# microsoft/protnote

Hardware: AMD Instinct MI355X
Metric: protein-label pairs/sec (fwd+bwd) (higher is better)
Workload: dtype f32

## Files before the change

### include/protnote_hip.h

```cpp
#ifndef PROTNOTE_HIP_H
#define PROTNOTE_HIP_H

#include <stddef.h>
#include <stdint.h>

#ifdef __cplusplus
extern "C" {
#endif

#define PN_MAX_BLOCKS 16
#define PN_MAX_LAYERS 8
#define PN_LABEL_F32 0
#define PN_LABEL_I64 1
#define PN_LABEL_U8 2

const char* pn_last_error(void);
int pn_version(void);
const char* pn_build_hash(void);

typedef struct pn_bn {
  const float* weight;
  const float* bias;
  float* running_mean;
  float* running_var;
// ... 179 lines not shown

#define PN_ADAM_WS_BYTES 32768
int pn_clip_adam_step(float* w, const float* g, float* m, float* v, long n, float max_norm, float lr, float beta1,
                      float beta2, float eps, float weight_decay, int step, float* norm_out, void* ws,
                      size_t ws_bytes, void* stream);

int pn_clip_sgd_step(float* w, const float* g, float* momentum_buf, long n, float max_norm, float lr, float momentum,
                     float weight_decay, int step, float* norm_out, void* ws, size_t ws_bytes, void* stream);

int pn_transpose(const float* src, long ld_src, int rows, int cols, float* dst, long ld_dst, void* stream);

int pn_gemm_tn(const float* A, long lda, const float* Bm, long ldb, float* C, long ldc, long R, int M, int N,
               void* ws, size_t ws_bytes, void* stream);

int pn_onehot_batch(const uint8_t* ids, const int64_t* offsets, int B, int A, int Lmax, float* onehots,
                    int64_t* lengths, void* stream);


int pn_ap_append(const float* scores, int ld_s, const void* labels, int label_kind, int ld_y, int B, int N_L,
                 uint32_t* keys, uint8_t* hits, long long cap, long long n0, void* stream);
size_t pn_ap_ws_bytes(int N_L, long long n, long long cap, int micro);
int pn_ap_compute(const uint32_t* keys, const uint8_t* hits, int N_L, long long n, long long cap, double* ap,
                  long long* npos, double* micro_ap, long long* micro_npos, void* ws, size_t ws_bytes, void* stream);

size_t pn_ap_partial_ws_bytes(long long m);
int pn_ap_partial(const uint32_t* keys, const uint8_t* hits, long long m, long long tp_before, long long k_before,
                  double* partial, long long* npos, void* ws, size_t ws_bytes, void* stream);

int pn_binned_hist_update(const float* scores, int ld_s, const void* labels, int label_kind, int ld_y, int B, int N_L,
                          const float* thresholds, int T, unsigned long long* pos_hist, unsigned long long* all_hist,
                          void* stream);
int pn_binned_auprc(unsigned long long* pos_hist, unsigned long long* all_hist, int N_L, int T, double* out,
                    long long* npos, int with_micro, void* stream);

int pn_set_math_mode(int mode);

int pn_set_mlp_materialize(int on);

typedef int (*pn_sync_hook)(long n_doubles, void* user);
int pn_set_sync_bn(pn_sync_hook hook, void* user, double* stage, long stage_doubles, int world);
int pn_get_math_mode(void);

int pn_set_backward_math(int mode);
int pn_get_backward_math(void);

int pn_set_forward_math(int mode);
int pn_get_forward_math(void);
int pn_set_fwd_staged(int on);
int pn_set_bf16_mfma16(int on);
int pn_set_bwd_deep(int mask);

int pn_set_f32_dma(int on);
int pn_set_b3_dma(int on);

int pn_set_encoder_f64(int on);

int pn_set_conv1_gather(int on);

int pn_dropout_mask(unsigned seed, int stream, float p, long rows, int cols, float* out, void* stream_);

int pn_prof_begin(void);
int pn_prof_end(int max_kinds, int* kinds, long* counts, double* total_ms, double* total_flops);

size_t pn_gemm_nt_stats_ws_bytes(int M, int N);
int pn_gemm_nt(const float* A, long lda, const float* W, long ldw, float* C, long ldc, int M, int N, int K,
               const float* bias, const float* a_scale, const float* a_shift, double* col_sum,
               double* col_sumsq, int tile_variant, void* ws, size_t ws_bytes, void* stream);

#ifdef __cplusplus
}
#endif
#endif
```

### protnote_amd/_lib.py

```python
import ctypes as C
import os

import torch

_HERE = os.path.dirname(os.path.abspath(__file__))
LIB_PATH = os.path.join(_HERE, "libprotnote_hip.so")

PN_MAX_BLOCKS = 16
PN_MAX_LAYERS = 8
PN_ADAM_WS_BYTES = 32768
fp = C.POINTER(C.c_float)


class pn_bn(C.Structure):
    _fields_ = [("weight", C.c_void_p), ("bias", C.c_void_p), ("running_mean", C.c_void_p),
                ("running_var", C.c_void_p)]


class pn_res_block(C.Structure):
    _fields_ = [("bn1", pn_bn), ("conv_a_w", C.c_void_p), ("conv_a_b", C.c_void_p), ("bn2", pn_bn),
                ("conv_b_w", C.c_void_p), ("conv_b_b", C.c_void_p)]


class pn_encoder(C.Structure):
# ... 108 lines not shown
    "pn_loss_fwd_bwd": (C.c_int, [C.c_void_p, C.c_void_p, C.c_void_p, C.c_int, C.c_int, C.c_int, C.c_float,
                                  C.c_float, C.c_float, C.c_float, C.c_float, C.c_void_p, C.c_void_p, C.c_void_p,
                                  C.c_void_p, C.c_void_p, C.c_int, C.c_void_p, C.c_float, C.c_void_p, C.c_size_t,
                                  C.c_void_p]),
    "pn_loss_fwd_bwd_t": (C.c_int, [C.c_void_p, C.c_void_p, C.c_int, C.c_int, C.c_int, C.c_int, C.c_float,
                                    C.c_float, C.c_float, C.c_float, C.c_float, C.c_void_p, C.c_void_p, C.c_void_p,
                                    C.c_void_p, C.c_void_p, C.c_int, C.c_void_p, C.c_float, C.c_void_p, C.c_size_t,
                                    C.c_void_p]),
    "pn_tp_fn_fp_t": (C.c_int, [C.c_void_p, C.c_void_p, C.c_int, C.c_int, C.c_int, C.c_float, C.c_void_p,
                                C.c_void_p, C.c_void_p, C.c_void_p]),
    "pn_supcon_ws_bytes": (C.c_size_t, [C.c_int]),
    "pn_supcon_fwd_bwd": (C.c_int, [C.c_void_p, C.c_void_p, C.c_void_p, C.c_int, C.c_int, C.c_void_p, C.c_void_p,
                                    C.c_void_p, C.c_size_t, C.c_void_p]),
    "pn_tp_fn_fp": (C.c_int, [C.c_void_p, C.c_void_p, C.c_void_p, C.c_int, C.c_int, C.c_float, C.c_void_p,
                              C.c_void_p, C.c_void_p, C.c_void_p]),
    "pn_clip_adam_step": (C.c_int, [C.c_void_p, C.c_void_p, C.c_void_p, C.c_void_p, C.c_long, C.c_float, C.c_float,
                                    C.c_float, C.c_float, C.c_float, C.c_float, C.c_int, C.c_void_p, C.c_void_p,
                                    C.c_size_t, C.c_void_p]),
    "pn_clip_sgd_step": (C.c_int, [C.c_void_p, C.c_void_p, C.c_void_p, C.c_long, C.c_float, C.c_float, C.c_float,
                                   C.c_float, C.c_int, C.c_void_p, C.c_void_p, C.c_size_t, C.c_void_p]),
    "pn_transpose": (C.c_int, [C.c_void_p, C.c_long, C.c_int, C.c_int, C.c_void_p, C.c_long, C.c_void_p]),
    "pn_gemm_tn": (C.c_int, [C.c_void_p, C.c_long, C.c_void_p, C.c_long, C.c_void_p, C.c_long, C.c_long, C.c_int,
                             C.c_int, C.c_void_p, C.c_size_t, C.c_void_p]),
    "pn_onehot_batch": (C.c_int, [C.c_void_p, C.c_void_p, C.c_int, C.c_int, C.c_int, C.c_void_p, C.c_void_p,
                                  C.c_void_p]),
    "pn_ap_append": (C.c_int, [C.c_void_p, C.c_int, C.c_void_p, C.c_int, C.c_int, C.c_int, C.c_int, C.c_void_p,
                               C.c_void_p, C.c_longlong, C.c_longlong, C.c_void_p]),
    "pn_ap_ws_bytes": (C.c_size_t, [C.c_int, C.c_longlong, C.c_longlong, C.c_int]),
    "pn_ap_compute": (C.c_int, [C.c_void_p, C.c_void_p, C.c_int, C.c_longlong, C.c_longlong, C.c_void_p, C.c_void_p,
                                C.c_void_p, C.c_void_p, C.c_void_p, C.c_size_t, C.c_void_p]),
    "pn_ap_partial_ws_bytes": (C.c_size_t, [C.c_longlong]),
    "pn_ap_partial": (C.c_int, [C.c_void_p, C.c_void_p, C.c_longlong, C.c_longlong, C.c_longlong, C.c_void_p, C.c_void_p,
                                C.c_void_p, C.c_size_t, C.c_void_p]),
    "pn_binned_hist_update": (C.c_int, [C.c_void_p, C.c_int, C.c_void_p, C.c_int, C.c_int, C.c_int, C.c_int,
                                        C.c_void_p, C.c_int, C.c_void_p, C.c_void_p, C.c_void_p]),
    "pn_binned_auprc": (C.c_int, [C.c_void_p, C.c_void_p, C.c_int, C.c_int, C.c_void_p, C.c_void_p, C.c_int,
                                  C.c_void_p]),
    "pn_dropout_mask": (C.c_int, [C.c_uint, C.c_int, C.c_float, C.c_long, C.c_int, C.c_void_p, C.c_void_p]),
    "pn_set_math_mode": (C.c_int, [C.c_int]),
    "pn_set_mlp_materialize": (C.c_int, [C.c_int]),
    "pn_set_sync_bn": (C.c_int, [C.c_void_p, C.c_void_p, C.c_void_p, C.c_long, C.c_int]),
    "pn_get_math_mode": (C.c_int, []),
    "pn_set_backward_math": (C.c_int, [C.c_int]),
    "pn_get_backward_math": (C.c_int, []),
    "pn_set_forward_math": (C.c_int, [C.c_int]),
    "pn_get_forward_math": (C.c_int, []),
    "pn_set_fwd_staged": (C.c_int, [C.c_int]),
    "pn_set_bf16_mfma16": (C.c_int, [C.c_int]),
    "pn_set_bwd_deep": (C.c_int, [C.c_int]),
    "pn_set_f32_dma": (C.c_int, [C.c_int]),
    "pn_set_encoder_f64": (C.c_int, [C.c_int]),
    "pn_set_conv1_gather": (C.c_int, [C.c_int]),
    "pn_set_b3_dma": (C.c_int, [C.c_int]),
    "pn_prof_begin": (C.c_int, []),
    "pn_prof_end": (C.c_int, [C.c_int, C.POINTER(C.c_int), C.POINTER(C.c_long), C.POINTER(C.c_double),
                              C.POINTER(C.c_double)]),
    "pn_gemm_nt": (C.c_int, [C.c_void_p, C.c_long, C.c_void_p, C.c_long, C.c_void_p, C.c_long, C.c_int, C.c_int,
                             C.c_int, C.c_void_p, C.c_void_p, C.c_void_p, C.c_void_p, C.c_void_p, C.c_int,
                             C.c_void_p, C.c_size_t, C.c_void_p]),
    "pn_gemm_nt_stats_ws_bytes": (C.c_size_t, [C.c_int, C.c_int]),
    "pn_loss_ws_bytes": (C.c_size_t, [C.c_int, C.c_int]),
}


def exported_symbols():
    return sorted(_SIGS)


def _ensure_current():
    from . import build

    have_src = os.path.isdir(build.CSRC) and os.path.exists(os.path.join(build.CSRC, "protnote_hip.hip"))
    if os.path.exists(LIB_PATH) and (not have_src or os.environ.get("PN_SKIP_HASH_CHECK") == "1"):
        return
    if os.path.exists(LIB_PATH) and not build.stale():
        return
    why = "is missing" if not os.path.exists(LIB_PATH) else (
        f"was built from other sources (binary {build.embedded_hash()}, csrc/ {build.csrc_hash()})")
    if not build.have_hipcc():
        raise RuntimeError(f"{LIB_PATH} {why} and hipcc is not available to rebuild it; build it with "
                           "`python -m protnote_amd.build` (protnote_amd has no CPU/eager fallback)")
    try:
        build.build_lib(verbose=False)
    except Exception as exc:
        raise RuntimeError(f"{LIB_PATH} {why} and could not be rebuilt ({exc}); build it with "
                           "`python -m protnote_amd.build` (protnote_amd has no CPU/eager fallback)") from exc


def build_hash() -> str:
    return lib().pn_build_hash().decode()


def lib():
    global _lib
    if _lib is None:
        _ensure_current()
        l = C.CDLL(LIB_PATH)
        for name, (res, args) in _SIGS.items():
            fn = getattr(l, name)
            fn.restype = res
            fn.argtypes = args
        _lib = l
        mode = os.environ.get("PN_MATH_MODE")
        if mode:
            set_math_mode(mode)
        mode = os.environ.get("PN_BACKWARD_MATH")
# ... 135 lines not shown
```

### protnote_amd/csrc/abi_heads_eval.hpp

```cpp
extern "C" size_t pn_mlp_rows_ws_bytes(const pn_mlp* m, int rows) {
  size_t b = 0;
  int hmax = 0;
  for (int i = 0; i + 1 < m->nlayers; ++i) hmax = m->dims[i + 1] > hmax ? m->dims[i + 1] : hmax;
  b += 2 * al256((size_t)rows * hmax * sizeof(float));
  b += 2 * al256((size_t)hmax * sizeof(float));
  return b;
}

extern "C" int pn_mlp_rows_fwd_eval(const pn_mlp* m, const float* x, int ldx, int rows, float* y, void* ws,
                                    size_t ws_bytes, void* stream) {
  PN_OK(math_field_check(m->math_mode, "pn_mlp_rows_fwd_eval"));
  MathScope math_scope(m->math_mode);
  hipStream_t st = (hipStream_t)stream;
  if (m->nlayers < 1 || m->nlayers > PN_MAX_LAYERS) return fail("mlp: bad layer count %d", m->nlayers);
  for (int i = 0; i <= m->nlayers; ++i)
    if (i < m->nlayers && m->dims[i] % 4 != 0) return fail("mlp: dims[%d]=%d not a multiple of 4", i, m->dims[i]);
  if (ldx % 4 != 0) return fail("mlp: ldx %% 4 != 0");
  int hmax = 0;
  for (int i = 0; i + 1 < m->nlayers; ++i) hmax = m->dims[i + 1] > hmax ? m->dims[i + 1] : hmax;
  Bump bp(ws, ws_bytes);
  float* buf[2];
  buf[0] = bp.take<float>((size_t)rows * hmax);
  buf[1] = bp.take<float>((size_t)rows * hmax);
  float* s = bp.take<float>(hmax);
// ... 442 lines not shown
    long rps = (p.R + ns - 1) / ns;
    p.rows_per_split = (rps + 31) / 32 * 32;
    ns = (int)((p.R + p.rows_per_split - 1) / p.rows_per_split);
  }
  const unsigned tiles = (unsigned)((p.M / 256) * (p.N / 256));
  dim3 grid(tiles, (unsigned)ns);
  p.task_ns = 0;
  int* sync_ws = p.task_sync;
  p.task_sync = nullptr;
  if (p.M == 3072 && p.N == 3072 && ns >= 2) {
    p.task_ns = ns;
    grid = dim3(tn_task_grid(ns), 1);
    if (SYNC && sync_ws != nullptr && ns * 4 * 4 <= TN_SYNC_INTS) {
      HIP_OK(hipMemsetAsync(sync_ws, 0, (size_t)ns * 4 * 4 * sizeof(int), st));
      p.task_sync = sync_ws;
    }
  }
  {
    ProfScope ps(100 + TA_PLAIN * 10 + TB, 2.0 * (double)R_all * (double)p.M * (double)p.N, st);
    hipLaunchKernelGGL(kern, grid, dim3(512), TN_FAST_LDS_BYTES, st, p);
    if (tail != 0) {
      auto tk = gemm_tn_kernel<TA_PLAIN, TB, false>;
      static bool tattr[64] = {false};
      if (dev < 64 && !tattr[dev]) {
        HIP_OK(hipFuncSetAttribute((const void*)tk, hipFuncAttributeMaxDynamicSharedMemorySize, TN_LDS_BYTES));
        tattr[dev] = true;
      }
      TnParams t = p;
      t.R = R_all; t.row_base = R_all - tail; t.rows_per_split = 32;
      t.Cpart = part + (size_t)ns * p.M * p.N; t.ldc = p.N; t.task_ns = 0; t.task_sync = nullptr;
      hipLaunchKernelGGL(tk, dim3((unsigned)((p.M / 128) * (p.N / 128)), 1), dim3(256), TN_LDS_BYTES, st, t);
    }
  }
  HIP_OK(hipGetLastError());
  if (ns > 1 || tail != 0) {
    hipLaunchKernelGGL(k_splitk_reduce, dim3(nblk((long)p.M * p.N, 256)), dim3(256), 0, st, (const float*)part,
                       ns + (tail != 0 ? 1 : 0), p.M, p.N, (long)p.N, dst, ldd);
    HIP_OK(hipGetLastError());
  }
  return 0;
}

template <int TB, int NP = 3, bool TR = false, bool ABF16 = false>
static int launch_tn_bf16x3(TnParams p, float* dst, long ldd, float* part, size_t part_cap_floats, hipStream_t st) {
  void (*kern)(TnParams) = nullptr;
  constexpr bool SYNC = TR && TB == TB_AFFINE_RELU;
  void (*kern_alt)(TnParams) = nullptr;
  if constexpr (TR) {
    kern = gemm_tn_bf16tr_kernel<TB, ABF16, SYNC, true>;
    kern_alt = gemm_tn_bf16tr_kernel<TB, ABF16, SYNC, false>;
  } else {
    kern = gemm_tn_bf16x3_kernel<TB, NP>;
  }
  constexpr int LDS = TR ? TN_BF16TR_LDS_BYTES : 2 * 512 * 36 * (int)sizeof(float);
  static std::atomic<bool> attr_done[64];
  int dev = 0;
  HIP_OK(hipGetDevice(&dev));
  if (dev < 64 && !attr_done[dev]) {
    HIP_OK(hipFuncSetAttribute((const void*)kern, hipFuncAttributeMaxDynamicSharedMemorySize, LDS));
    if (kern_alt != nullptr) HIP_OK(hipFuncSetAttribute((const void*)kern_alt, hipFuncAttributeMaxDynamicSharedMemorySize, LDS));
    attr_done[dev] = true;
  }
  if (kern_alt != nullptr && !g_bf16_m16.load()) kern = kern_alt;
  int ns = tn_pick_split(p.R, p.M, p.N, part_cap_floats, 256, 1);
  if (ns == 1) {
    p.Cpart = dst;
    p.ldc = ldd;
    p.rows_per_split = (p.R + 31) / 32 * 32;
  } else {
    if (part == nullptr) return fail("gemm_tn: no partial buffer");
    p.Cpart = part;
    p.ldc = p.N;
    long rps = (p.R + ns - 1) / ns;
    p.rows_per_split = (rps + 31) / 32 * 32;
    ns = (int)((p.R + p.rows_per_split - 1) / p.rows_per_split);
  }
  const unsigned tiles = (unsigned)((p.M / 256) * (p.N / 256));
  dim3 grid(tiles, (unsigned)ns);
  p.task_ns = 0;
  int* sync_ws = p.task_sync;
  p.task_sync = nullptr;
  if (p.M == 3072 && p.N == 3072 && ns >= 2) {
    p.task_ns = ns;
    grid = dim3(tn_task_grid(ns), 1);
    if (SYNC && sync_ws != nullptr && ns * 4 * 4 <= TN_SYNC_INTS) {
      HIP_OK(hipMemsetAsync(sync_ws, 0, (size_t)ns * 4 * 4 * sizeof(int), st));
      p.task_sync = sync_ws;
    }
  }
  {
    ProfScope ps((NP == 3 ? 1100 : 1600) + TB, 2.0 * (double)p.R * (double)p.M * (double)p.N, st);
    hipLaunchKernelGGL(kern, grid, dim3(512), LDS, st, p);
  }
  HIP_OK(hipGetLastError());
  if (ns > 1) {
    hipLaunchKernelGGL(k_splitk_reduce, dim3(nblk((long)p.M * p.N, 256)), dim3(256), 0, st, (const float*)part, ns,
                       p.M, p.N, (long)p.N, dst, ldd);
    HIP_OK(hipGetLastError());
  }
  return 0;
}

template <int TA, int TB>
static int launch_tn(TnParams p, float* dst, long ldd, float* part, size_t part_cap_floats, hipStream_t st) {
  if (p.M % 4 || p.N % 4) return fail("gemm_tn: M and N must be multiples of 4");
  if (p.R <= 0) return fail("gemm_tn: empty contraction");
  if (p.drop_thresh != 0) {
    if constexpr (TA == TA_PLAIN && (TB == TB_AFFINE_RELU || TB == TB_PAIRSUM_RELU)) {
      if (PN_BIG && use_f32_dma() && p.M % 256 == 0 && p.N % 256 == 0 && p.R >= 65536 && p.R % 32 == 0 && p.lda % 4 == 0)
        return launch_tn_cfg<TA, TB, true, true, true>(p, dst, ldd, part, part_cap_floats, st);
      return launch_tn_cfg<TA, TB, false, false, true>(p, dst, ldd, part, part_cap_floats, st);
    } else {
      return fail("gemm_tn: dropout is not defined for operand kinds %d x %d", TA, TB);
    }
  }
  if constexpr (TA == TA_PLAIN && (TB == TB_AFFINE_RELU || TB == TB_PAIRSUM_RELU)) {
// ... 59 lines not shown
```

### protnote_amd/csrc/protnote_hip.hip

```cpp
#include <hip/hip_runtime.h>
#include <stdarg.h>
#include <stdio.h>
#include <stdlib.h>
#include <string.h>

#include "../../include/protnote_hip.h"
#include "common.hpp"
#include "gemm_engine.hpp"
#include "gemm_bf16x3.hpp"
#include "gemm_bf16.hpp"
#include "gemm_dma.hpp"
#include "gemm_conv_dma.hpp"
#include "gemm_conv_f64.hpp"
#include "gemm_tn_fast.hpp"
#include "train_kernels.hpp"
#include "bwd_bf16_dz.hpp"
#include "fwd_bf16_h.hpp"
#include "gemm_bf16_m16.hpp"

using namespace pn;

static thread_local char g_err[512] = "";

static int fail(const char* fmt, ...) {
  va_list ap;
  va_start(ap, fmt);
  vsnprintf(g_err, sizeof(g_err), fmt, ap);
  va_end(ap);
  return 1;
}

#define HIP_OK(expr)                                                                         \
  do {                                                                                       \
    hipError_t _e = (expr);                                                                  \
    if (_e != hipSuccess) return fail("%s failed: %s (%s:%d)", #expr, hipGetErrorString(_e), \
                                      __FILE__, __LINE__);                                   \
  } while (0)
#define PN_OK(expr)         \
  do {                      \
    int _r = (expr);        \
    if (_r != 0) return _r; \
  } while (0)

int pn::fail_msg(const char* fmt, ...) {
  va_list ap;
  va_start(ap, fmt);
  vsnprintf(g_err, sizeof(g_err), fmt, ap);
  va_end(ap);
  return 1;
}

extern "C" const char* pn_last_error(void) { return g_err; }
extern "C" int pn_version(void) { return 1; }

static inline int ld4(int c) { return (c + 3) & ~3; }
static inline size_t al256(size_t b) { return (b + 255) & ~(size_t)255; }

struct Bump {
  char* base;
  size_t off, cap;
  bool ok;
  Bump(void* p, size_t cap_) : base((char*)p), off(0), cap(cap_), ok(true) {}
  template <class T>
  T* take(size_t n) {
    size_t b = al256(n * sizeof(T));
    if (off + b > cap) {
      ok = false;
      return nullptr;
    }
    T* r = (T*)(base + off);
    off += b;
// ... 255 lines not shown
  return 0;
}

static std::atomic<int> g_bwd_math{0};
extern "C" int pn_set_backward_math(int mode) {
  if (mode != 0 && mode != 1) return fail("pn_set_backward_math: 0 (as the forward) or 1 (bf16, one product)");
  g_bwd_math = mode;
  return 0;
}
extern "C" int pn_get_backward_math(void) { return g_bwd_math; }
static thread_local bool tl_bwd_bf16 = false;
static thread_local bool tl_dz_bf16 = false;
struct BwdBf16Scope {
  bool prev;
  explicit BwdBf16Scope(bool on) : prev(tl_bwd_bf16) { tl_bwd_bf16 = on; }
  ~BwdBf16Scope() {
    tl_bwd_bf16 = prev;
    tl_dz_bf16 = false;
  }
};

static std::atomic<int> g_fwd_math{0};
extern "C" int pn_set_forward_math(int mode) {
  if (mode != 0 && mode != 1) return fail("pn_set_forward_math: 0 (as math_mode) or 1 (bf16, one product)");
  g_fwd_math = mode;
  return 0;
}
extern "C" int pn_get_forward_math(void) { return g_fwd_math; }
static thread_local bool tl_fwd_bf16 = false;
struct FwdBf16Scope {
  bool prev;
  explicit FwdBf16Scope(bool on) : prev(tl_fwd_bf16) { tl_fwd_bf16 = on; }
  ~FwdBf16Scope() { tl_fwd_bf16 = prev; }
};
static bool fwd_bf16_requested(const pn_pairhead* hd) {
  const int m = hd->forward_math == 0 ? g_fwd_math.load(std::memory_order_relaxed) : hd->forward_math - 1;
  return m == 1 && hd->dropout_p == 0.f;
}
static int fwd_math_of(const pn_pairhead* hd, bool* bf16) {
  if (hd->forward_math < 0 || hd->forward_math > 2)
    return fail("pairhead: forward_math %d (0 = library default, 1 = as math_mode, 2 = bf16)", hd->forward_math);
  const int m = hd->forward_math == 0 ? g_fwd_math.load(std::memory_order_relaxed) : hd->forward_math - 1;
  *bf16 = (m == 1) && hd->dropout_p == 0.f;
  return 0;
}

static std::atomic<int> g_b3_dma{1};
static bool use_b3_dma() { return g_b3_dma == 1; }
extern "C" int pn_set_b3_dma(int on) {
  g_b3_dma = on ? 1 : 0;
  return 0;
}

template <int AK, int EK, int WAVES_N, int WN, bool GEN, bool BDMA = false, int NP = 3>
static int launch_gemm_bf16x3(const GemmParams& p, hipStream_t st) {
  using Cfg = GemmCfg<4, WAVES_N, 2, WN, 32>;
  if constexpr (!GEN && !BDMA && WAVES_N * WN * 32 == 256) {
    if (p.wsplit != nullptr && use_b3_dma() && p.Nstore == p.N)
      return launch_gemm_bf16x3<AK, EK, WAVES_N, WN, GEN, true>(p, st);
  }
  auto kern = gemm_nt_bf16x3_kernel<AK, EK, 4, WAVES_N, 2, WN, GEN, BDMA, NP>;
  constexpr int LDS_BYTES = BDMA ? 2 * (256 * 36 + 2 * 256 * 16) * (int)sizeof(float) : Cfg::LDS_BYTES;
  static std::atomic<bool> attr_done[64];
  int dev = 0;
  HIP_OK(hipGetDevice(&dev));
  if (dev < 64 && !attr_done[dev]) {
    HIP_OK(hipFuncSetAttribute((const void*)kern, hipFuncAttributeMaxDynamicSharedMemorySize, LDS_BYTES));
    attr_done[dev] = true;
  }
  if (p.M <= 0 || p.Nstore <= 0) return 0;
  if (p.Kseg % 4 != 0) return fail("gemm: K segment %d not a multiple of 4", p.Kseg);
  const long tm = (p.M + Cfg::BM - 1) / Cfg::BM;
  const long tn = (p.Nstore + Cfg::BN - 1) / Cfg::BN;
  GemmParams pp = p;
  pp.xcd_bc = (PN_XCD && tm >= 16) ? ((tn % 8 == 0) ? 8 : ((tn % 4 == 0) ? 4 : 0)) : 0;
  if (!GEN && AK == A_PAIRSUM_RELU && pp.xcd_bc && tm >= 64) pp.xcd_bc = 1;
  pp.xcd_br = pp.xcd_bc ? 32 / pp.xcd_bc : 0;
  long grid = tm * tn;
  if (pp.xcd_bc) {
    const long nblk = ((tm + pp.xcd_br - 1) / pp.xcd_br) * (tn / pp.xcd_bc);
    grid = ((nblk + 7) / 8) * 8 * 32;
  }
  if (grid > 0x7fffffffL) return fail("gemm: grid too large");
  if constexpr (BDMA) {
    pp.w_hi = p.wsplit;
    pp.w_lo = p.wsplit + (size_t)p.N * p.Kseg;
    hipLaunchKernelGGL(k_split_planes, dim3(nblk((long)p.N * p.Kseg / 4, 256)), dim3(256), 0, st, p.W, p.ldw, p.N, p.Kseg,
                       p.wsplit, p.wsplit + (size_t)p.N * p.Kseg);
  }
  {
    ProfScope ps((NP == 3 ? 1000 : 1500) + AK * 10 + EK, 2.0 * (double)p.M * (double)p.N * (double)p.nseg * (double)p.Kseg, st);
    hipLaunchKernelGGL(kern, dim3((unsigned)grid), dim3(Cfg::NT), LDS_BYTES, st, pp);
  }
  HIP_OK(hipGetLastError());
  return finish_col_stats(p, tm, st);
}

static std::atomic<int> g_bwd_deep{7};
extern "C" int pn_set_bwd_deep(int mask) {
  g_bwd_deep = mask & 7;
  return 0;
}
static int launch_gemm_bf16_single(const GemmParams& p, hipStream_t st) {
  auto kern = gemm_nt_bf16_kernel<E_STORE>;
  static std::atomic<bool> attr_done[64];
  int dev = 0;
  HIP_OK(hipGetDevice(&dev));
  if (dev < 64 && !attr_done[dev]) {
    HIP_OK(hipFuncSetAttribute((const void*)kern, hipFuncAttributeMaxDynamicSharedMemorySize, NT_BF16_LDS_BYTES));
    attr_done[dev] = true;
  }
  if (p.M <= 0 || p.Nstore <= 0) return 0;
  const long tm = (p.M + 255) / 256, tn = p.N / 256;
  GemmParams pp = p;
  pp.xcd_bc = (PN_XCD && tm >= 16) ? ((tn % 8 == 0) ? 8 : ((tn % 4 == 0) ? 4 : 0)) : 0;
  pp.xcd_br = pp.xcd_bc ? 32 / pp.xcd_bc : 0;
  long grid = tm * tn;
  if (pp.xcd_bc) {
    const long nblk_ = ((tm + pp.xcd_br - 1) / pp.xcd_br) * (tn / pp.xcd_bc);
    grid = ((nblk_ + 7) / 8) * 8 * 32;
  }
// ... 518 lines not shown
```

Measured before the change: 1.249 million.

## Add 16x16x32 bf16 MFMA variants of bf16x3 NT and TN GEMM kernels

Adds new bf16x3 (split hi/lo) GEMM kernels for the NT (with B DMA) and TN paths. They use 16x16x32 bf16 MFMA instructions instead of 32x32, with a new swizzled LDS layout, interleaved instruction scheduling, and permlane swaps that convert the accumulators back to 32x32 layout for the existing epilogue. A new default mode picks the new kernel only for plain-A NT GEMMs and pairsum-relu TN GEMMs. The aim is higher MFMA throughput and better overlap of loads with compute, at the cost of extra permute work and more code complexity.

```diff
diff --git a/include/protnote_hip.h b/include/protnote_hip.h
--- a/include/protnote_hip.h
+++ b/include/protnote_hip.h
@@ -255,6 +255,8 @@
 
 int pn_set_f32_dma(int on);
 int pn_set_b3_dma(int on);
+int pn_set_b3_mfma16(int on);
+int pn_get_b3_mfma16(void);
 
 int pn_set_encoder_f64(int on);
 
diff --git a/protnote_amd/_lib.py b/protnote_amd/_lib.py
--- a/protnote_amd/_lib.py
+++ b/protnote_amd/_lib.py
@@ -184,6 +184,8 @@
     "pn_set_encoder_f64": (C.c_int, [C.c_int]),
     "pn_set_conv1_gather": (C.c_int, [C.c_int]),
     "pn_set_b3_dma": (C.c_int, [C.c_int]),
+    "pn_set_b3_mfma16": (C.c_int, [C.c_int]),
+    "pn_get_b3_mfma16": (C.c_int, []),
     "pn_prof_begin": (C.c_int, []),
     "pn_prof_end": (C.c_int, [C.c_int, C.POINTER(C.c_int), C.POINTER(C.c_long), C.POINTER(C.c_double),
                               C.POINTER(C.c_double)]),
diff --git a/protnote_amd/csrc/abi_heads_eval.hpp b/protnote_amd/csrc/abi_heads_eval.hpp
--- a/protnote_amd/csrc/abi_heads_eval.hpp
+++ b/protnote_amd/csrc/abi_heads_eval.hpp
@@ -518,16 +518,24 @@
   } else {
     kern = gemm_tn_bf16x3_kernel<TB, NP>;
   }
-  constexpr int LDS = TR ? TN_BF16TR_LDS_BYTES : 2 * 512 * 36 * (int)sizeof(float);
+  int LDS = TR ? TN_BF16TR_LDS_BYTES : 2 * 512 * 36 * (int)sizeof(float);
   static std::atomic<bool> attr_done[64];
   int dev = 0;
   HIP_OK(hipGetDevice(&dev));
   if (dev < 64 && !attr_done[dev]) {
     HIP_OK(hipFuncSetAttribute((const void*)kern, hipFuncAttributeMaxDynamicSharedMemorySize, LDS));
     if (kern_alt != nullptr) HIP_OK(hipFuncSetAttribute((const void*)kern_alt, hipFuncAttributeMaxDynamicSharedMemorySize, LDS));
+    if constexpr (!TR && NP == 3)
+      HIP_OK(hipFuncSetAttribute((const void*)gemm_tn_b3m16_kernel<TB>, hipFuncAttributeMaxDynamicSharedMemorySize, B3M16_LDS_BYTES));
     attr_done[dev] = true;
   }
   if (kern_alt != nullptr && !g_bf16_m16.load()) kern = kern_alt;
+  if constexpr (!TR && NP == 3) {
+    if (b3_m16_tn(TB)) {
+      kern = gemm_tn_b3m16_kernel<TB>;
+      LDS = B3M16_LDS_BYTES;
+    }
+  }
   int ns = tn_pick_split(p.R, p.M, p.N, part_cap_floats, 256, 1);
   if (ns == 1) {
     p.Cpart = dst;
diff --git a/protnote_amd/csrc/gemm_bf16x3_m16.hpp b/protnote_amd/csrc/gemm_bf16x3_m16.hpp
--- /dev/null
+++ b/protnote_amd/csrc/gemm_bf16x3_m16.hpp
@@ -0,0 +1,485 @@
+#pragma once
+#include "gemm_bf16x3.hpp"
+
+#ifndef PN_B3M16_VALU
+#define PN_B3M16_VALU 3
+#endif
+
+namespace pn {
+
+constexpr int B3M16_ROWF = 32;
+constexpr int B3M16_TILE = 256 * B3M16_ROWF;
+constexpr int B3M16_STAGE = 2 * B3M16_TILE;
+constexpr int B3M16_LDS_BYTES = 2 * B3M16_STAGE * (int)sizeof(float);
+
+__device__ __forceinline__ int b3m16_swz(int r) { return ((r >> 1) & 7) ^ ((r & 1) << 2); }
+
+__device__ __forceinline__ void b3m16_frag_offsets(int lane, int wm, int wn, int (&fa)[3], int (&fb)[3]) {
+  const int frow = lane & 15, q = lane >> 4, lowq = q < 2;
+  const int sw = b3m16_swz(frow);
+  const int sa[3] = {(q & 1) | (lowq ? 4 : 0), lowq ? q : 4 + q, 2 + (q & 1)};
+  const int sb[3] = {lowq ? q : 2 + q, q, lowq ? 6 + q : q};
+#pragma unroll
+  for (int t = 0; t < 3; ++t) {
+    fa[t] = (wm * 64 + frow) * B3M16_ROWF + 4 * (sa[t] ^ sw);
+    fb[t] = B3M16_TILE + (wn * 128 + frow) * B3M16_ROWF + 4 * (sb[t] ^ sw);
+  }
+}
+
+template <int T>
+__device__ __forceinline__ void b3m16_step(const float* stage, const int (&fa)[3], const int (&fb)[3], f32x4 (&acc)[4][8]) {
+  bf16x8 a[4], b[8];
+#pragma unroll
+  for (int i = 0; i < 4; ++i) a[i] = *reinterpret_cast<const bf16x8*>(stage + fa[T] + i * 16 * B3M16_ROWF);
+#pragma unroll
+  for (int j = 0; j < 8; ++j) b[j] = *reinterpret_cast<const bf16x8*>(stage + fb[T] + j * 16 * B3M16_ROWF);
+#pragma unroll
+  for (int i = 0; i < 4; ++i)
+#pragma unroll
+    for (int j = 0; j < 8; ++j) acc[i][j] = __builtin_amdgcn_mfma_f32_16x16x32_bf16(a[i], b[j], acc[i][j], 0, 0, 0);
+}
+
+__device__ __forceinline__ void b3m16_store8(float* image, int r, int g, float4 v0, float4 v1) {
+  const HiLo a = split4(v0), b = split4(v1);
+  bf16x8 hi, lo;
+#pragma unroll
+  for (int e = 0; e < 4; ++e) {
+    hi[e] = a.hi[e];
+    hi[4 + e] = b.hi[e];
+    lo[e] = a.lo[e];
+    lo[4 + e] = b.lo[e];
+  }
+  const int sw = b3m16_swz(r & 15);
+  *reinterpret_cast<bf16x8*>(image + r * B3M16_ROWF + 4 * (g ^ sw)) = hi;
+  *reinterpret_cast<bf16x8*>(image + r * B3M16_ROWF + 4 * ((4 + g) ^ sw)) = lo;
+}
+
+__device__ __forceinline__ void acc16_to_acc32(const f32x4 (&a)[4][8], f32x16 (&o)[2][4]) {
+#pragma unroll
+  for (int i = 0; i < 4; ++i)
+#pragma unroll
+    for (int j = 0; j < 4; ++j)
+#pragma unroll
+      for (int e = 0; e < 4; ++e) {
+        const float f0 = a[i][2 * j][e], f1 = a[i][2 * j + 1][e];
+        const auto s = __builtin_amdgcn_permlane16_swap(__float_as_uint(f0), __float_as_uint(f1), false, false);
+        const auto t = __builtin_amdgcn_permlane32_swap(s[0], s[1], false, false);
+        o[i >> 1][j][e + 8 * (i & 1)] = __uint_as_float(t[0]);
+        o[i >> 1][j][e + 8 * (i & 1) + 4] = __uint_as_float(t[1]);
+      }
+}
+
+template <int AK, int EK>
+__global__ __launch_bounds__(512, 2) void gemm_nt_b3m16_kernel(const GemmParams p) {
+  static_assert(AK == A_PLAIN || AK == A_AFFINE_RELU || AK == A_PAIRSUM_RELU, "operand kind not built for bf16x3");
+  constexpr int BM = 256, BN = 256, BK = 32;
+  constexpr int WAVES_M = 4, WAVES_N = 2;
+  constexpr int RPP = 128;
+  constexpr int NQA = BM / RPP;
+  constexpr int STAGE = B3M16_STAGE;
+
+  extern __shared__ __attribute__((aligned(16))) float smem[];
+
+  const int tid = threadIdx.x;
+  const int lane = tid & 63;
+  const int wave = tid >> 6;
+  const int wm = wave / WAVES_N;
+  const int wn = wave % WAVES_N;
+
+  int tile_m, tile_n;
+  if (!tile_coords<BM, BN>(p, tile_m, tile_n)) return;
+  const int row0 = tile_m * BM;
+  const int col0 = tile_n * BN;
+
+  const uint16_t* bsrc[4];
+  unsigned bdst[4];
+  {
+    const int w = __builtin_amdgcn_readfirstlane(wave);
+#pragma unroll
+    for (int q = 0; q < 4; ++q) {
+      const int c = 4 * w + q;
+      const int r = 8 * c + (lane >> 3);
+      const int slot = (lane & 7) ^ b3m16_swz(r & 15);
+      bsrc[q] = ((slot >> 2) ? p.w_lo : p.w_hi) + (long)(col0 + r) * p.Kseg + 8 * (slot & 3);
+      bdst[q] = (unsigned)(B3M16_TILE + 8 * c * B3M16_ROWF) * 4u;
+    }
+  }
+  const unsigned lds0_b = (unsigned)(uintptr_t)(const __attribute__((address_space(3))) float*)smem;
+  auto issue_b_dma = [&](int s_, int buf) {
+#pragma unroll
+    for (int q = 0; q < 4; ++q)
+      tn_glds16(reinterpret_cast<const float*>(bsrc[q] + s_ * BK),
+                __builtin_amdgcn_readfirstlane(lds0_b + (unsigned)(buf * STAGE) * 4u + bdst[q]));
+  };
+
+  const int kv = tid & 3;
+  const int r_in = tid >> 2;
+
+  const float* arow[NQA];
+  const float* arow2[NQA];
+#pragma unroll
+  for (int q = 0; q < NQA; ++q) {
+    int r = row0 + r_in + q * RPP;
+    if (r > p.M - 1) r = p.M - 1;
+    if constexpr (AK == A_PAIRSUM_RELU) {
+      const int j = r / p.pairB;
+      const int i = r - j * p.pairB;
+      arow[q] = p.A + (long)i * p.lda + 4 * kv;
+      arow2[q] = p.A2 + (long)j * p.lda2 + 4 * kv;
+    } else {
+      arow[q] = p.A + (long)r * p.lda + 4 * kv;
+      arow2[q] = nullptr;
+    }
+  }
+
+  const int nslab = p.Kseg / BK;
+
+  float4 ra[NQA][2], ra2[NQA][2];
+  float4 rsc[2], rsh[2];
+
+  auto fetch_a = [&](int s) {
+    const int c = s * BK;
+#pragma unroll
+    for (int q = 0; q < NQA; ++q)
+#pragma unroll
+      for (int h = 0; h < 2; ++h) {
+        ra[q][h] = ld4(arow[q] + c + 16 * h);
+        if constexpr (AK == A_PAIRSUM_RELU) ra2[q][h] = ld4(arow2[q] + c + 16 * h);
+      }
+    if constexpr (AK == A_AFFINE_RELU) {
+#pragma unroll
+      for (int h = 0; h < 2; ++h) {
+        rsc[h] = ld4(p.a_scale + c + 4 * kv + 16 * h);
+        rsh[h] = ld4(p.a_shift + c + 4 * kv + 16 * h);
+      }
+    }
+  };
+  auto pin_a = [&]() {
+#pragma unroll
+    for (int q = 0; q < NQA; ++q)
+#pragma unroll
+      for (int h = 0; h < 2; ++h) {
+        pin4(ra[q][h]);
+        if constexpr (AK == A_PAIRSUM_RELU) pin4(ra2[q][h]);
+      }
+  };
+  auto commit_a = [&](int buf) {
+    float* As = smem + buf * STAGE;
+#pragma unroll
+    for (int q = 0; q < NQA; ++q) {
+      float4 v[2];
+#pragma unroll
+      for (int h = 0; h < 2; ++h) {
+        v[h] = ra[q][h];
+        if constexpr (AK == A_AFFINE_RELU) {
+          v[h].x = relu(fmaf(v[h].x, rsc[h].x, rsh[h].x));
+          v[h].y = relu(fmaf(v[h].y, rsc[h].y, rsh[h].y));
+          v[h].z = relu(fmaf(v[h].z, rsc[h].z, rsh[h].z));
+          v[h].w = relu(fmaf(v[h].w, rsc[h].w, rsh[h].w));
+        } else if constexpr (AK == A_PAIRSUM_RELU) {
+          v[h].x = relu(v[h].x + ra2[q][h].x);
+          v[h].y = relu(v[h].y + ra2[q][h].y);
+          v[h].z = relu(v[h].z + ra2[q][h].z);
+          v[h].w = relu(v[h].w + ra2[q][h].w);
+        }
+      }
+      b3m16_store8(As, r_in + q * RPP, kv, v[0], v[1]);
+    }
+  };
+
+  f32x4 acc[4][8];
+#pragma unroll
+  for (int i = 0; i < 4; ++i)
+#pragma unroll
+    for (int j = 0; j < 8; ++j)
+#pragma unroll
+      for (int e = 0; e < 4; ++e) acc[i][j][e] = 0.f;
+
+  int fa[3], fb[3];
+  b3m16_frag_offsets(lane, wm, wn, fa, fb);
+
+  auto weave = [&](auto nvalu_c) {
+    constexpr int NV = decltype(nvalu_c)::value;
+    __builtin_amdgcn_sched_group_barrier(0x100, 12, 0);
+#pragma unroll
+    for (int i = 0; i < 32; ++i) {
+      __builtin_amdgcn_sched_group_barrier(0x008, 1, 0);
+      __builtin_amdgcn_sched_group_barrier(0x002, NV, 0);
+      if (i % 8 == 7) __builtin_amdgcn_sched_group_barrier(0x200, 1, 0);
+    }
+  };
+
+  using std::integral_constant;
+  issue_b_dma(0, 0);
+  fetch_a(0);
+  pin_a();
+  commit_a(0);
+  fetch_a(nslab > 1 ? 1 : 0);
+  asm volatile("s_waitcnt vmcnt(0) lgkmcnt(0)" ::: "memory");
+  __builtin_amdgcn_s_barrier();
+  for (int s = 0; s + 1 < nslab; ++s) {
+    const int cur = s & 1;
+    const int nxt = s + 2 < nslab ? s + 2 : s + 1;
+    const float* stage = smem + cur * STAGE;
+    __builtin_amdgcn_sched_barrier(0);
+    pin_a();
+    issue_b_dma(s + 1, cur ^ 1);
+    __builtin_amdgcn_sched_barrier(0);
+    b3m16_step<0>(stage, fa, fb, acc);
+    commit_a(cur ^ 1);
+    weave(integral_constant<int, (AK == A_PLAIN ? PN_B3M16_VALU : PN_B3M16_VALU + 1)>{});
+    __builtin_amdgcn_sched_barrier(0);
+    asm volatile("s_waitcnt vmcnt(0)" ::: "memory");
+    fetch_a(nxt);
+    __builtin_amdgcn_sched_barrier(0);
+    b3m16_step<1>(stage, fa, fb, acc);
+    b3m16_step<2>(stage, fa, fb, acc);
+    __builtin_amdgcn_sched_barrier(0);
+    asm volatile("s_waitcnt lgkmcnt(0)" ::: "memory");
+    __builtin_amdgcn_s_barrier();
+  }
+  {
+    const float* stage = smem + ((nslab - 1) & 1) * STAGE;
+    b3m16_step<0>(stage, fa, fb, acc);
+    b3m16_step<1>(stage, fa, fb, acc);
+    b3m16_step<2>(stage, fa, fb, acc);
+  }
+  __syncthreads();
+
+  f32x16 acc32[2][4];
+  acc16_to_acc32(acc, acc32);
+  gemm_epilogue<EK, WAVES_M, WAVES_N, 2, 4>(p, acc32, row0, col0, tile_n, smem);
+}
+
+template <int TB>
+__global__ __launch_bounds__(512, 2) void gemm_tn_b3m16_kernel(const TnParams p) {
+  constexpr int BM = 256, BN = 256, BK = 32;
+  constexpr int STAGE = B3M16_STAGE;
+  static_assert(TB == TB_PLAIN || TB == TB_AFFINE_RELU || TB == TB_PAIRSUM_RELU, "operand kind not built for bf16x3");
+
+  extern __shared__ __attribute__((aligned(16))) float smem[];
+
+  const int tid = threadIdx.x;
+  const int lane = tid & 63;
+  const int wave = tid >> 6;
+  const int wm = wave >> 1, wn = wave & 1;
+
+  const int ntn = p.N / BN, ntm = p.M / BM;
+  int tile_m, tile_n;
+  int split = blockIdx.y;
+  if (p.task_ns > 0) {
+    if (!tn_task_coords(p.task_ns, tile_m, tile_n, split)) return;
+  } else if (PN_XCD && TB == TB_PAIRSUM_RELU && (ntm % 4 == 0) && (ntn % 2 == 0)) {
+    const int rm = ntm / 4, rn = ntn / 2;
+    const int xcd = blockIdx.x & 7, w = blockIdx.x >> 3;
+    tile_m = (xcd >> 1) * rm + w / rn;
+    tile_n = (xcd & 1) * rn + w % rn;
+  } else if (PN_XCD && (ntm % 2 == 0) && (ntn % 4 == 0)) {
+    const int rm = ntm / 2, rn = ntn / 4;
+    const int xcd = blockIdx.x & 7, w = blockIdx.x >> 3;
+    tile_m = (xcd >> 2) * rm + w / rn;
+    tile_n = (xcd & 3) * rn + w % rn;
+  } else {
+    tile_n = blockIdx.x % ntn;
+    tile_m = blockIdx.x / ntn;
+  }
+  const int m0 = tile_m * BM, n0 = tile_n * BN;
+  const long r_begin = (long)split * p.rows_per_split;
+  long r_end = r_begin + p.rows_per_split;
+  if (r_end > p.R) r_end = p.R;
+
+  const int col = tid & 255;
+  const int kg = __builtin_amdgcn_readfirstlane(tid >> 8);
+  float bs = 0.f, bt = 0.f;
+  if constexpr (TB == TB_AFFINE_RELU) {
+    bs = p.b_s[n0 + col];
+    bt = p.b_t[n0 + col];
+  }
+
+  float ra[2][8], rb[2][8], rb2[2];
+  const unsigned pB = (unsigned)p.pairB;
+  const long lda = p.lda, ldb = p.ldb;
+
+  auto fetch_a = [&](long k0, auto safe_c) {
+    constexpr bool SAFE = decltype(safe_c)::value;
+    const float* Ak = p.A + k0 * lda + m0;
+    const int lim = (int)(r_end - 1 - k0);
+#pragma unroll
+    for (int g = 0; g < 2; ++g)
+#pragma unroll
+      for (int e = 0; e < 8; ++e) {
+        int ro = 8 * (kg + 2 * g) + e;
+        if (SAFE) ro = ro < lim ? ro : lim;
+        const float* rowp = Ak + (long)ro * lda;
+        ra[g][e] = rowp[(unsigned)col];
+      }
+  };
+  auto fetch_b = [&](long k0, auto safe_c) {
+    constexpr bool SAFE = decltype(safe_c)::value;
+    const int lim = (int)(r_end - 1 - k0);
+    if constexpr (TB == TB_PAIRSUM_RELU) {
+#pragma unroll
+      for (int g = 0; g < 2; ++g) {
+        int rr0 = 8 * (kg + 2 * g);
+        if (SAFE) rr0 = rr0 < lim ? rr0 : (lim & ~7);
+        const unsigned ru = (unsigned)(k0 + rr0);
+        const unsigned j = ru / pB;
+        const unsigned i = ru - j * pB;
+        const float* Bi = p.B + (long)i * ldb + n0;
+#pragma unroll
+        for (int e = 0; e < 8; ++e) {
+          int eo = e;
+          if (SAFE) eo = (rr0 + e) < lim ? e : (lim - rr0 > 0 ? lim - rr0 : 0);
+          const float* rowp = Bi + (long)eo * ldb;
+          rb[g][e] = rowp[(unsigned)col];
+        }
+        const float* B2j = p.B2 + (long)j * p.ldb2 + n0;
+        rb2[g] = B2j[(unsigned)col];
+      }
+    } else {
+      const float* Bk = p.B + k0 * ldb + n0;
+#pragma unroll
+      for (int g = 0; g < 2; ++g)
+#pragma unroll
+        for (int e = 0; e < 8; ++e) {
+          int ro = 8 * (kg + 2 * g) + e;
+          if (SAFE) ro = ro < lim ? ro : lim;
+          const float* rowp = Bk + (long)ro * ldb;
+          rb[g][e] = rowp[(unsigned)col];
+        }
+    }
+  };
+
+  auto pin_a = [&]() {
+#pragma unroll
+    for (int g = 0; g < 2; ++g)
+#pragma unroll
+      for (int e = 0; e < 8; ++e) asm volatile("" : "+v"(ra[g][e]));
+  };
+  auto pin_b = [&]() {
+#pragma unroll
+    for (int g = 0; g < 2; ++g) {
+#pragma unroll
+      for (int e = 0; e < 8; ++e) asm volatile("" : "+v"(rb[g][e]));
+      if constexpr (TB == TB_PAIRSUM_RELU) asm volatile("" : "+v"(rb2[g]));
+    }
+  };
+
+  auto commit_a = [&](int buf, long k0, auto safe_c) {
+    constexpr bool SAFE = decltype(safe_c)::value;
+    float* As = smem + buf * STAGE;
+#pragma unroll
+    for (int g = 0; g < 2; ++g) {
+      float a[8];
+#pragma unroll
+      for (int e = 0; e < 8; ++e) {
+        a[e] = ra[g][e];
+        if (SAFE && k0 + 8 * (kg + 2 * g) + e >= r_end) a[e] = 0.f;
+      }
+      b3m16_store8(As, col, kg + 2 * g, make_float4(a[0], a[1], a[2], a[3]), make_float4(a[4], a[5], a[6], a[7]));
+    }
+  };
+  auto commit_b = [&](int buf, long k0, auto safe_c) {
+    constexpr bool SAFE = decltype(safe_c)::value;
+    float* Bs = smem + buf * STAGE + B3M16_TILE;
+#pragma unroll
+    for (int g = 0; g < 2; ++g) {
+      float b[8];
+#pragma unroll
+      for (int e = 0; e < 8; ++e) {
+        b[e] = rb[g][e];
+        if constexpr (TB == TB_AFFINE_RELU) b[e] = relu(fmaf(b[e], bs, bt));
+        if constexpr (TB == TB_PAIRSUM_RELU) b[e] = relu(b[e] + rb2[g]);
+        if (SAFE && k0 + 8 * (kg + 2 * g) + e >= r_end) b[e] = 0.f;
+      }
+      b3m16_store8(Bs, col, kg + 2 * g, make_float4(b[0], b[1], b[2], b[3]), make_float4(b[4], b[5], b[6], b[7]));
+    }
+  };
+
+  f32x4 acc[4][8];
+#pragma unroll
+  for (int i = 0; i < 4; ++i)
+#pragma unroll
+    for (int j = 0; j < 8; ++j)
+#pragma unroll
+      for (int e = 0; e < 4; ++e) acc[i][j][e] = 0.f;
+
+  int fa[3], fb[3];
+  b3m16_frag_offsets(lane, wm, wn, fa, fb);
+
+  using std::integral_constant;
+  using std::false_type;
+  using std::true_type;
+  auto weave = [&](auto nvalu_c) {
+    constexpr int NV = decltype(nvalu_c)::value;
+    __builtin_amdgcn_sched_group_barrier(0x100, 12, 0);
+#pragma unroll
+    for (int i = 0; i < 32; ++i) {
+      __builtin_amdgcn_sched_group_barrier(0x008, 1, 0);
+      __builtin_amdgcn_sched_group_barrier(0x002, NV, 0);
+      if (i % 8 == 7) __builtin_amdgcn_sched_group_barrier(0x200, 1, 0);
+    }
+  };
+  if (r_begin < r_end) {
+    const long span = r_end - r_begin;
+    const int nf = (int)(span / BK);
+    const int ns = nf + ((span % BK) ? 1 : 0);
+    auto K0 = [&](int t) { return r_begin + (long)t * BK; };
+    auto body = [&](int t, auto safe_c) {
+      const int cur = t & 1;
+      const int t2 = t + 2 < ns ? t + 2 : t + 1;
+      const float* stage = smem + cur * STAGE;
+      __builtin_amdgcn_sched_barrier(0);
+      pin_a();
+      b3m16_step<0>(stage, fa, fb, acc);
+      commit_a(cur ^ 1, K0(t + 1), safe_c);
+      weave(integral_constant<int, 2>{});
+      __builtin_amdgcn_sched_barrier(0);
+      fetch_a(K0(t2), safe_c);
+      __builtin_amdgcn_sched_barrier(0);
+      pin_b();
+      b3m16_step<1>(stage, fa, fb, acc);
+      commit_b(cur ^ 1, K0(t + 1), safe_c);
+      weave(integral_constant<int, 2>{});
+      __builtin_amdgcn_sched_barrier(0);
+      fetch_b(K0(t2), safe_c);
+      __builtin_amdgcn_sched_barrier(0);
+      b3m16_step<2>(stage, fa, fb, acc);
+      __syncthreads();
+    };
+    fetch_a(K0(0), true_type{});
+    fetch_b(K0(0), true_type{});
+    pin_a();
+    pin_b();
+    commit_a(0, K0(0), true_type{});
+    commit_b(0, K0(0), true_type{});
+    fetch_a(K0(ns > 1 ? 1 : 0), true_type{});
+    fetch_b(K0(ns > 1 ? 1 : 0), true_type{});
+    __syncthreads();
+    int t = 0;
+    for (; t + 2 < nf; ++t) body(t, false_type{});
+    for (; t + 1 < ns; ++t) body(t, true_type{});
+    const float* stage = smem + ((ns - 1) & 1) * STAGE;
+    b3m16_step<0>(stage, fa, fb, acc);
+    b3m16_step<1>(stage, fa, fb, acc);
+    b3m16_step<2>(stage, fa, fb, acc);
+  }
+
+  f32x16 acc32[2][4];
+  acc16_to_acc32(acc, acc32);
+  float* out = p.Cpart + (long)split * p.M * p.ldc;
+  const int hl = lane >> 5, cl = lane & 31;
+#pragma unroll
+  for (int i = 0; i < 2; ++i)
+#pragma unroll
+    for (int j = 0; j < 4; ++j) {
+      const int n = n0 + (wn * 4 + j) * 32 + cl;
+#pragma unroll
+      for (int e = 0; e < 16; ++e) {
+        const int m = m0 + (wm * 2 + i) * 32 + (e & 3) + 8 * (e >> 2) + 4 * hl;
+        out[(long)m * p.ldc + n] = acc32[i][j][e];
+      }
+    }
+}
+
+}
diff --git a/protnote_amd/csrc/protnote_hip.hip b/protnote_amd/csrc/protnote_hip.hip
--- a/protnote_amd/csrc/protnote_hip.hip
+++ b/protnote_amd/csrc/protnote_hip.hip
@@ -17,6 +17,7 @@
 #include "bwd_bf16_dz.hpp"
 #include "fwd_bf16_h.hpp"
 #include "gemm_bf16_m16.hpp"
+#include "gemm_bf16x3_m16.hpp"
 
 using namespace pn;
 
@@ -378,6 +379,22 @@
   return 0;
 }
 
+static std::atomic<int> g_b3_m16{4};
+extern "C" int pn_set_b3_mfma16(int on) {
+  if (on < 0 || on > 4) return fail("pn_set_b3_mfma16: 0 (32x32x16), 1 (16x16x32), 2 (NT only), 3 (TN only) or 4 (measured-best per kernel)");
+  g_b3_m16 = on;
+  return 0;
+}
+extern "C" int pn_get_b3_mfma16(void) { return g_b3_m16.load(); }
+static bool b3_m16_nt(int ak) {
+  const int m = g_b3_m16.load();
+  return m == 4 ? ak == A_PLAIN : (m == 1 || m == 2);
+}
+static bool b3_m16_tn(int tb) {
+  const int m = g_b3_m16.load();
+  return m == 4 ? tb == TB_PAIRSUM_RELU : (m == 1 || m == 3);
+}
+
 template <int AK, int EK, int WAVES_N, int WN, bool GEN, bool BDMA = false, int NP = 3>
 static int launch_gemm_bf16x3(const GemmParams& p, hipStream_t st) {
   using Cfg = GemmCfg<4, WAVES_N, 2, WN, 32>;
@@ -385,14 +402,23 @@
     if (p.wsplit != nullptr && use_b3_dma() && p.Nstore == p.N)
       return launch_gemm_bf16x3<AK, EK, WAVES_N, WN, GEN, true>(p, st);
   }
-  auto kern = gemm_nt_bf16x3_kernel<AK, EK, 4, WAVES_N, 2, WN, GEN, BDMA, NP>;
-  constexpr int LDS_BYTES = BDMA ? 2 * (256 * 36 + 2 * 256 * 16) * (int)sizeof(float) : Cfg::LDS_BYTES;
+  void (*kern)(GemmParams) = gemm_nt_bf16x3_kernel<AK, EK, 4, WAVES_N, 2, WN, GEN, BDMA, NP>;
+  int LDS_BYTES = BDMA ? 2 * (256 * 36 + 2 * 256 * 16) * (int)sizeof(float) : Cfg::LDS_BYTES;
+  constexpr bool HAS_M16 = BDMA && NP == 3;
   static std::atomic<bool> attr_done[64];
   int dev = 0;
   HIP_OK(hipGetDevice(&dev));
   if (dev < 64 && !attr_done[dev]) {
     HIP_OK(hipFuncSetAttribute((const void*)kern, hipFuncAttributeMaxDynamicSharedMemorySize, LDS_BYTES));
+    if constexpr (HAS_M16)
+      HIP_OK(hipFuncSetAttribute((const void*)gemm_nt_b3m16_kernel<AK, EK>, hipFuncAttributeMaxDynamicSharedMemorySize, B3M16_LDS_BYTES));
     attr_done[dev] = true;
+  }
+  if constexpr (HAS_M16) {
+    if (b3_m16_nt(AK)) {
+      kern = gemm_nt_b3m16_kernel<AK, EK>;
+      LDS_BYTES = B3M16_LDS_BYTES;
+    }
   }
   if (p.M <= 0 || p.Nstore <= 0) return 0;
   if (p.Kseg % 4 != 0) return fail("gemm: K segment %d not a multiple of 4", p.Kseg);
```

Measured after the change: 1.249 million, median of 6. No clear change (+0.0%).
